# eanswer/TactileSimulation

Measured on AMD Instinct MI355X. Metric: env-steps/sec (fwd+bwd) TactilePush batch=4096, higher is better.
Workload: dtype f32

## Files before the change

### include/tsim.h

```cpp
#ifndef TSIM_H
#define TSIM_H
#include <stdint.h>
#ifdef __cplusplus
extern "C" {
#endif

typedef struct tsim_batch tsim_batch;
enum { TSIM_F32 = 0, TSIM_F64 = 1 };

int tsim_batch_create(const int32_t* I, const double* F, int B, int tape_capacity, int dtype, int device,
                      tsim_batch** out);
void tsim_batch_destroy(tsim_batch* b);

int tsim_ndof_r(const tsim_batch* b);
int tsim_ndof_u(const tsim_batch* b);
int tsim_ndof_var(const tsim_batch* b);
int tsim_ndof_tactile(const tsim_batch* b);
int tsim_batch_size(const tsim_batch* b);
int tsim_dtype(const tsim_batch* b);
double tsim_timestep(const tsim_batch* b);
int tsim_tape_len(const tsim_batch* b);

int tsim_update_model(tsim_batch* b, const int32_t* I, const double* F, void* stream);

// ... 43 lines not shown
enum { TSIM_PARAM_JACOBIAN_MAX_COLS = 32 };
int tsim_param_jacobians(tsim_batch* b, int num_frames, int num_steps, int ncols, const int32_t* cols,
                         const int32_t* tactile_slot, void* E_out, void* Ft_out, void* stream);
int tsim_param_jacobians_launch_info(const tsim_batch* b, int32_t* out);

int tsim_tactile_normal_equations(tsim_batch* b, int num_frames, int num_steps, const int32_t* tactile_slot, int with_params,
                                  const void* weight, const void* resid, void* N_out, void* n_out, void* stream);
int tsim_tactile_normal_equations_launch_info(const tsim_batch* b, int with_params, int32_t* out);

int tsim_get_adjoint(tsim_batch* b, void* df_dq0, void* df_dqd0, void* stream);

int tsim_cache_save(tsim_batch* b, void* stream);
int tsim_cache_pop(tsim_batch* b, void* stream);
int tsim_cache_clear(tsim_batch* b);
int tsim_cache_reserve(tsim_batch* b, int depth);
int tsim_cache_depth(const tsim_batch* b);

int tsim_debug_eval(tsim_batch* b, const void* q1, const void* q0, const void* qd0, const void* u,
                    void* g_out, void* H_out, long long* cycles, void* stream);

int tsim_debug_signature(tsim_batch* b, int t_first, int n, uint32_t* out, void* stream);

int tsim_debug_stamps(tsim_batch* b, long long* cycles);

int tsim_launch_info(const tsim_batch* b, int32_t* out);
enum { TSIM_KT_FORWARD = 0, TSIM_KT_TAXELS = 1, TSIM_KT_BACKWARD = 2, TSIM_KT_COUNT = 3 };
int tsim_kernel_timing(tsim_batch* b, int enable);
int tsim_kernel_times(tsim_batch* b, double* ms_sum, int32_t* launches);
int tsim_set_lanes_per_env(tsim_batch* b, int lanes);
int tsim_static_model(const tsim_batch* b);
int tsim_set_static(tsim_batch* b, int allow);
const char* tsim_kernel_variant(const tsim_batch* b);
enum { TSIM_OPT_PAIR_CULL = 1, TSIM_OPT_VALUE_TRIALS = 2, TSIM_OPT_TRIAL_HELPERS = 3, TSIM_OPT_VALUE_FIRST = 4, TSIM_OPT_CROSS_KINKS = 5, TSIM_OPT_EVAL_BUDGET = 6,
       TSIM_OPT_ALL_DEFAULT = 7, TSIM_OPT_FRAME_RECORDS = 8, TSIM_OPT_FORWARD_SPLIT = 9, TSIM_OPT_PREDICTOR_HELPERS = 10, TSIM_OPT_ADJOINT_PREPASS = 11 };
int tsim_set_option(tsim_batch* b, int option, int value);
int tsim_get_option(const tsim_batch* b, int option);

int tsim_last_evals(tsim_batch* b, int32_t* host_out);
int tsim_last_helper_trials(tsim_batch* b, int32_t* host_out);

#define TSIM_KINK_FACTOR 1000.0
#define TSIM_KINK_LS 4
#define TSIM_KINK_MAX 6
int tsim_set_solver_options(tsim_batch* b, int cross_kinks, int eval_budget);
int tsim_last_gnorm(tsim_batch* b, float* host_out);

const char* tsim_last_error(void);

#ifdef __cplusplus
}
#endif
#endif
```

### tactilesimulation_amd/csrc/tsim_batch.h

```cpp
#pragma once
#include <hip/hip_runtime.h>
#include <cstdint>
#include <string>
#include <vector>
#include "../../include/tsim.h"
#include "tsim_launch.h"

static thread_local std::string g_err;
static int fail(const std::string& m) { g_err = m; return 1; }
#define HIPCHK(x) do { hipError_t e_ = (x); if (e_ != hipSuccess) return fail(std::string(#x) + ": " + hipGetErrorString(e_)); } while (0)

struct DeviceGuard {
  int prev = -1; bool ok = true;
  explicit DeviceGuard(int dev) {
    if (hipGetDevice(&prev) != hipSuccess) prev = -1;
    if (prev != dev) ok = hipSetDevice(dev) == hipSuccess; else prev = -1;
  }
  ~DeviceGuard() { if (prev >= 0) (void)hipSetDevice(prev); }
};
#define TS_DEVICE(b) DeviceGuard guard_((b)->device); if (!guard_.ok) return fail("hipSetDevice(" + std::to_string((b)->device) + ") failed")

static bool capturing(hipStream_t st) {
  hipStreamCaptureStatus cs = hipStreamCaptureStatusNone;
  return hipStreamIsCapturing(st, &cs) != hipSuccess || cs != hipStreamCaptureStatusNone;
}

template <class F> static auto by_dtype(int dtype, F&& f) { return dtype == TSIM_F32 ? f(float()) : f(double()); }

struct DevBuf {
  void* p = nullptr;
  DevBuf() = default;
  DevBuf(const DevBuf&) = delete;
  DevBuf& operator=(const DevBuf&) = delete;
  ~DevBuf() { (void)hipFree(p); }
  template <class U> operator U*() const { return static_cast<U*>(p); }
  explicit operator bool() const { return p != nullptr; }
  void** operator&() { return &p; }
  void* take() { void* q = p; p = nullptr; return q; }
  void release() { (void)hipFree(take()); }
};

struct CacheEntry { void* buf; int len; int record, tape_k_ok; };
struct KtPair { hipEvent_t a, b; int kind; };
struct tsim_batch {
  int B, dtype, device, cap;
  std::vector<int32_t> I; std::vector<double> F;
  int nl, nr, nu, nvar, ntax, rec;
  int tape_k = 0, tape_k_ok = 0;
  DevBuf dI, dF;
  DevBuf dFenv; int nfrec;
  void* tape = nullptr;
  DevBuf lamq, lamv;
  DevBuf evals;
  DevBuf helped;
  DevBuf gnorm;
  int cross_kinks = 0, eval_budget = 0;
  DevBuf order; int order_valid = 0;
  DevBuf order_ep; int order_ep_n = 0;
  DevBuf prev; int has_prev = 0;
  DevBuf poseR, poseD; int nspt;
  int has_exp;
  int t_cur, record;
  int lpe_forced;
  int nsched;
  int stage_cpt;
  int n_simd;
  int last_frame_rec = 0;
  hipStream_t split_st = nullptr;
  hipEvent_t split_fork = nullptr;
  hipEvent_t split_join = nullptr;
  int last_fwd_split = 0;
  int value_trials = 2;
  int pred_helpers = 1;
  int trial_helpers = 1;
  int value_first = 1;
  bool ab_no_episode_lpt = false, ab_inkernel_readout = false, ab_no_free_run = false, ab_lockstep = false, ab_taxels_per_record = false, ab_no_envtab_cpt = false, ab_no_default_opts = false, ab_inkernel_frame_out = false; int ab_bwd_lpe = 0, ab_lpt_deal = 2;
  int pair_cull = 1;
  int static_id = 0, static_exact = 0, env_struct_ok = 0, no_static = 0;
  DevBuf dKmask, dFlag;
  DevBuf fposeR, fposeD; int fpose_frames = 0;
  int pose_valid = 0;
  int pose_off = 0;
  int tt_off = 0;
  int tax_slots = 0;
  size_t esz;
  std::vector<CacheEntry> cache;
// ... 59 lines not shown
```

### tactilesimulation_amd/csrc/tsim_hip.hip

```cpp
#include <hip/hip_runtime.h>
#include <cstdio>
#include <cstdlib>
#include <cstring>
#include <cmath>
#include <algorithm>
#include <string>
#include <vector>
#include "../../include/tsim.h"
#include "tsim_eval.h"
#include "tsim_policy_push.h"
#include "tsim_static_pusher.h"


#include "tsim_kernels.h"
#include "tsim_param_grad.h"
#include "tsim_launch.h"
#include "tsim_adjoint_pre.h"
#include "tsim_batch.h"

__global__ void __launch_bounds__(1024) k_order_by_evals(const int* evals, int* order, int B, int ns, int lo, int span, int deal) {
  __shared__ int hist[64], base[64];
  const int t = threadIdx.x;
  if (t < 64) hist[t] = 0;
  __syncthreads();
// ... 607 lines not shown
  HIPCHK(hipGetLastError());
  return 0;
}

template <class R>
static int launch_forward(tsim_batch* b, const void* u, int nframes, const int32_t* tac_slot, int nsub, void* q_out, void* qd_out, void* var_out, void* tac_out, int32_t* status, hipStream_t st) {
  FwdArgs<R> a = fwd_args<R>(b);
  a.nsub = nsub; a.nframes = nframes; a.tac_slot = tac_slot; a.u = (const R*)u;
  a.q_out = (R*)q_out; a.qd_out = (R*)qd_out; a.var_out = (R*)var_out; a.tac_out = (R*)tac_out; a.status = status;
  a.order = (b->B >= 256 && nframes == 1 && b->order_valid) ? (const int*)b->order : (b->B >= 256 && nframes > 1 && b->order_ep_n == nframes * nsub && !b->ab_no_episode_lpt) ? (const int*)b->order_ep : nullptr;
  a.vo_first = b->value_first; a.helpers = b->trial_helpers; a.helped = b->helped;
  a.pred_helpers = b->trial_helpers && b->pred_helpers;
  const bool emit = pose_emit(b, st);
  a.nspt = b->nspt;
  if (emit) { a.poseR = (R*)b->poseR; a.poseD = b->poseD; }
  const size_t fpose_bytes = (size_t)nframes * b->B * (size_t)std::max(b->nspt, 1) * (TP_R_SIZE * b->esz + TP_D_SIZE * sizeof(double));
  bool defer = tac_out && taxels_supported(b) && fpose_bytes <= ((size_t)1 << 30) && !b->ab_inkernel_readout;
  if (defer && b->fpose_frames < nframes) {
    if (capturing(st)) defer = false;
    else {
      const size_t nrec = (size_t)nframes * b->B * b->nspt;
      const int rc = grow_buffers(b, st, b->pose_off != 0, {{b->fposeR, nrec * TP_R_SIZE * b->esz}, {b->fposeD, nrec * TP_D_SIZE * sizeof(double)}});
      if (rc > 0) return rc;
      b->fpose_frames = rc ? 0 : nframes;
      if (rc) defer = false;
    }
  }
  if (defer) { a.fposeR = (R*)b->fposeR; a.fposeD = b->fposeD; }
  a.free_run = (defer || !tac_out || b->ntax == 0) && !b->ab_no_free_run;
  a.lockstep = b->ab_lockstep ? 1 : 0;
  if (a.lockstep) a.free_run = 0;
  TsPlan plan = ts_plan(b, TS_K_FORWARD, false, 0);
  if (b->record && !plan.fused) b->tape_k_ok = 0;
  const TsPlan fr_plan = ts_plan(b, TS_K_FRAME_RECORDS, false, 0);
  const bool frame_rec = defer && a.free_run && b->record && nframes > 1 && plan.fused && !emit && !b->ab_inkernel_frame_out &&
                         fr_plan.variant == plan.variant && fr_plan.lpe == plan.lpe;
  a.frame_rec = frame_rec ? 1 : 0;
  plan.frame_rec = frame_rec;
  b->last_frame_rec = !frame_rec ? 0 : (plan.frame_rec && plan.default_opts) ? 2 : 1;
  const int ns_ = TS_WAVE / plan.lpe;
  auto frame_records = [&](hipStream_t s, const TsSubRange& sub) {
    TsPlan p = fr_plan;
    const int nblk = (sub.n + ns_ - 1) / ns_, chunks = std::max(1, std::min(nframes, b->n_simd / std::max(nblk, 1))), fpc = (nframes + chunks - 1) / chunks;
    p.grid = (unsigned)(nblk * ((nframes + fpc - 1) / fpc));
    return ts_launch<false, R>(p, s, a, fpc, sub);
  };
  const int nblk_f = (int)plan.grid, wh = std::max(1, nblk_f / 8);
  const bool split = frame_rec && b->split_st && a.order && a.order == (const int*)b->order_ep && b->B % ns_ == 0 && nblk_f <= b->n_simd && nblk_f >= 64 &&
                     taxels_small(b, (long long)nframes * wh * ns_) && !capturing(st);
  b->last_fwd_split = split ? 1 : 0;
  if (split) {
    const TsSubRange heavy{a.order, 0, wh * ns_}, light{a.order, wh * ns_, b->B - wh * ns_};
    auto forward = [&](hipStream_t s, unsigned grid, const FwdArgs<R>& fa) -> int {
      TsPlan p = plan; p.grid = grid;
      if (!ts_launch<false, R>(p, s, fa)) return fail("no k_forward instantiation for the launch plan");
      HIPCHK(hipGetLastError());
      return 0;
    };
    auto read_out = [&](hipStream_t s, const TsSubRange& sub) -> int {
      if (!frame_records(s, sub)) return fail("no k_frame_records instantiation for the launch plan");
      HIPCHK(hipGetLastError());
      return launch_taxels<R>(b, b->fposeR, b->fposeD, nframes, tac_slot, tac_out, s, &sub);
    };
    int rc;
    {
      KtScope kt_(b, TSIM_KT_FORWARD, st);
      HIPCHK(hipEventRecord(b->split_fork, st));
      HIPCHK(hipStreamWaitEvent(b->split_st, b->split_fork, 0));
      rc = forward(st, (unsigned)wh, a);
    }
    if (!rc) {
      FwdArgs<R> al = a; al.order = a.order + light.e0;
// ... 277 lines not shown
  const int nl = I[TSIM_IH_NL], nr = I[TSIM_IH_NR], nu = I[TSIM_IH_NU];
  int n_exp = 0;
  if (nr > 16 || nr < 1 || nu > 16) return fail("ndof_r must be in 1..16 and ndof_u <= 16");
  for (int i = 1; i <= nl; ++i) {
    int jt = I[I[TSIM_IH_OFF_LINK] + (i - 1) * TSIM_LI_SIZE + TSIM_LI_JTYPE];
    if (jt != TSIM_J_REVOLUTE && jt != TSIM_J_PRISMATIC && jt != TSIM_J_PLANAR && jt != TSIM_J_TRANSLATIONAL && jt != TSIM_J_SPHERICAL_EXP)
      return fail("joint type not supported by the HIP path");
    if (jt == TSIM_J_SPHERICAL_EXP && ++n_exp > 1) return fail("at most one rotation-vector joint per model on the HIP path");
  }
  for (int s = 0; s < I[TSIM_IH_NSENSOR]; ++s)
    if (I[I[TSIM_IH_OFF_SENSOR] + s * TSIM_SI_SIZE + TSIM_SI_NSPRIM] > 16) return fail("too many primitives per sensor");
  DeviceGuard guard_(device);
  if (!guard_.ok) return fail("hipSetDevice(" + std::to_string(device) + ") failed");
  tsim_batch* b = new tsim_batch();
  b->B = B; b->dtype = dtype; b->device = device; b->cap = tape_capacity;
  b->I.assign(I, I + I[TSIM_IH_NI]); b->F.assign(F, F + I[TSIM_IH_NF]);
  b->nl = nl; b->nr = nr; b->nu = nu; b->nvar = I[TSIM_IH_NVAR]; b->ntax = I[TSIM_IH_NTAXEL];
  b->esz = dtype == TSIM_F32 ? 4 : 8;
  b->t_cur = 0; b->record = 0; b->has_exp = n_exp > 0;
  b->nfrec = I[TSIM_IH_FOFF_CPT];
  b->lpe_forced = 0;
  { const std::vector<int32_t> S_ = build_sched(b->I, b->F); b->nsched = (int)S_.size(); b->tt_off = b->I[TSIM_IH_NI] + S_[TS_SCHED_TAXTAB]; }
  b->pair_cull = getenv("TSIM_NO_PAIR_CULL") ? 0 : 1;
  b->no_static = getenv("TSIM_NO_STATIC") != nullptr;
  b->trial_helpers = getenv("TSIM_NO_TRIAL_HELPERS") ? 0 : 1;
  b->pred_helpers = getenv("TSIM_NO_PREDICTOR_HELPERS") ? 0 : 1;
  b->ab_no_episode_lpt = getenv("TSIM_NO_EPISODE_LPT") != nullptr; b->ab_inkernel_readout = getenv("TSIM_INKERNEL_READOUT") != nullptr;
  b->ab_no_free_run = getenv("TSIM_NO_FREE_RUN") != nullptr; b->ab_lockstep = getenv("TSIM_LOCKSTEP") != nullptr; b->ab_no_default_opts = getenv("TSIM_NO_DEFAULT_OPTS") != nullptr;
  if (const char* e = getenv("TSIM_LPT_DEAL")) b->ab_lpt_deal = atoi(e);
  if (const char* e = getenv("TSIM_BWD_LPE")) { const int v = atoi(e); if (v == 16 || v == 32 || v == 64) b->ab_bwd_lpe = v; }
  b->ab_taxels_per_record = getenv("TSIM_TAXELS_PER_RECORD") != nullptr; b->ab_no_envtab_cpt = getenv("TSIM_NO_ENVTAB_CPT") != nullptr;
  b->value_first = getenv("TSIM_NO_VALUE_FIRST") ? 0 : 1;
  b->ab_inkernel_frame_out = getenv("TSIM_INKERNEL_FRAME_OUT") != nullptr;
  if (const char* e = getenv("TSIM_VALUE_TRIALS")) b->value_trials = std::max(0, atoi(e));
  if (const char* e = getenv("TSIM_LPE")) { const int v = atoi(e); if (v == 16 || v == 32 || v == 64) b->lpe_forced = v; }
  b->cross_kinks = dtype == TSIM_F32 ? 1 : 0;
  {
    int cus = 0;
    if (hipDeviceGetAttribute(&cus, hipDeviceAttributeMultiprocessorCount, device) != hipSuccess || cus <= 0) cus = 256;
    b->n_simd = 4 * cus;
  }
  b->stage_cpt = 0;
  detect_static_model(b);
  b->tape_k = kernel_mode(b, b->lpe_forced) != TS_KM_GENERIC ? 1 : 0;
  b->rec = ts_rec(nr, nu, (int)b->esz, b->tape_k);
  if (lds_bytes_for(b, 1) > 64 * 1024) { delete b; return fail("model needs more than 64 KiB of LDS per environment"); }
  decide_stage_cpt(b);
  b->nspt = b->I[TSIM_IH_NSPRIM];
  size_t tape_bytes = (size_t)(tape_capacity + 1) * B * b->rec * b->esz;
  if (hipMalloc(&b->dI, (b->I.size() + b->nsched) * sizeof(int32_t)) != hipSuccess || hipMalloc(&b->dF, b->F.size() * b->esz) != hipSuccess ||
      hipMalloc(&b->tape, tape_bytes) != hipSuccess || hipMalloc(&b->lamq, (size_t)2 * B * nr * b->esz) != hipSuccess ||
      hipMalloc(&b->lamv, (size_t)2 * B * nr * b->esz) != hipSuccess || hipMalloc(&b->evals, (size_t)B * sizeof(int)) != hipSuccess || hipMalloc((void**)&b->helped, (size_t)B * sizeof(int)) != hipSuccess || hipMemset(b->helped, 0, (size_t)B * sizeof(int)) != hipSuccess || hipMalloc((void**)&b->gnorm, (size_t)B * sizeof(float)) != hipSuccess || hipMalloc(&b->order, (size_t)B * sizeof(int)) != hipSuccess || hipMalloc((void**)&b->order_ep, (size_t)B * sizeof(int)) != hipSuccess || hipMalloc(&b->prev, (size_t)B * 2 * nr * sizeof(double)) != hipSuccess ||
      (b->nspt > 0 && (hipMalloc(&b->poseR, (size_t)B * b->nspt * TP_R_SIZE * b->esz) != hipSuccess || hipMalloc((void**)&b->poseD, (size_t)B * b->nspt * TP_D_SIZE * sizeof(double)) != hipSuccess))) {
    tsim_batch_destroy(b);
    return fail("hipMalloc failed (tape bytes = " + std::to_string(tape_bytes) + ")");
  }
  if (hipMemset(b->tape, 0, tape_bytes) != hipSuccess || hipMemset(b->lamq, 0, (size_t)2 * B * nr * b->esz) != hipSuccess ||
      hipMemset(b->lamv, 0, (size_t)2 * B * nr * b->esz) != hipSuccess) { tsim_batch_destroy(b); return fail("hipMemset failed"); }
  if (upload_model(b, nullptr)) { tsim_batch_destroy(b); return 1; }
  b->adj_pre = getenv("TSIM_NO_ADJOINT_PREPASS") ? 0 : 1;
  if (b->adj_pre && b->tape_k && dtype == TSIM_F32 && tape_capacity > 0 && hipMalloc(&b->sseed, (size_t)tape_capacity * B * 2 * nr * b->esz) != hipSuccess) {
    (void)hipGetLastError();
    b->adj_pre = 0;
  }
  if (B >= 64 && !getenv("TSIM_NO_FORWARD_SPLIT")) {
    if (hipStreamCreateWithFlags(&b->split_st, hipStreamNonBlocking) != hipSuccess || hipEventCreateWithFlags(&b->split_fork, hipEventDisableTiming) != hipSuccess ||
// ... 73 lines not shown
int tsim_static_model(const tsim_batch* b) { return kernel_mode(b, b->lpe_forced) != TS_KM_GENERIC ? b->static_id : 0; }
const char* tsim_kernel_variant(const tsim_batch* b) {
  const int km = kernel_mode(b, b->lpe_forced);
  if (km == TS_KM_STATIC) return "static:pusher";
  if (km == TS_KM_PARAM) return "param:pusher";
  return "generic";
}
int tsim_set_static(tsim_batch* b, int allow) {
  b->no_static = allow ? 0 : 1;
  shape_changed(b);
  return 0;
}
int tsim_set_option(tsim_batch* b, int option, int value) {
  if (option == TSIM_OPT_PAIR_CULL) { b->pair_cull = value != 0; return 0; }
  if (option == TSIM_OPT_VALUE_TRIALS) { if (value < 0) return fail("set_option: TSIM_OPT_VALUE_TRIALS >= 0"); b->value_trials = value; return 0; }
  if (option == TSIM_OPT_TRIAL_HELPERS) { b->trial_helpers = value != 0; return 0; }
  if (option == TSIM_OPT_VALUE_FIRST) { b->value_first = value != 0; return 0; }
  if (option == TSIM_OPT_PREDICTOR_HELPERS) { b->pred_helpers = value != 0; return 0; }
  if (option == TSIM_OPT_ADJOINT_PREPASS) { b->adj_pre = value != 0; return 0; }
  return fail("set_option: unknown option " + std::to_string(option));
}
int tsim_get_option(const tsim_batch* b, int option) {
  if (option == TSIM_OPT_PAIR_CULL) return b->pair_cull;
  if (option == TSIM_OPT_VALUE_TRIALS) return b->value_trials;
  if (option == TSIM_OPT_TRIAL_HELPERS) return b->trial_helpers;
  if (option == TSIM_OPT_VALUE_FIRST) return b->value_first;
  if (option == TSIM_OPT_CROSS_KINKS) return b->cross_kinks;
  if (option == TSIM_OPT_EVAL_BUDGET) return b->eval_budget;
  if (option == TSIM_OPT_ALL_DEFAULT) return default_options(b) ? 1 : 0;
  if (option == TSIM_OPT_FRAME_RECORDS) return b->last_frame_rec;
  if (option == TSIM_OPT_FORWARD_SPLIT) return b->last_fwd_split;
  if (option == TSIM_OPT_PREDICTOR_HELPERS) return b->pred_helpers;
  if (option == TSIM_OPT_ADJOINT_PREPASS) return b->adj_pre_ran;
  return -1;
}
int tsim_set_solver_options(tsim_batch* b, int cross_kinks, int eval_budget) {
  if (eval_budget < 0) return fail("set_solver_options: negative evaluation budget");
  b->cross_kinks = cross_kinks != 0;
  b->eval_budget = eval_budget;
  return 0;
}
int tsim_last_gnorm(tsim_batch* b, float* host_out) {
  TS_DEVICE(b);
  if (hipMemcpy(host_out, b->gnorm, (size_t)b->B * sizeof(float), hipMemcpyDeviceToHost) != hipSuccess) return fail("last_gnorm: copy failed");
  return 0;
}
int tsim_last_helper_trials(tsim_batch* b, int32_t* host_out) {
  TS_DEVICE(b);
  if (hipMemcpy(host_out, b->helped, (size_t)b->B * sizeof(int), hipMemcpyDeviceToHost) != hipSuccess) return fail("last_helper_trials: copy failed");
  return 0;
}
int tsim_last_evals(tsim_batch* b, int32_t* host_out) {
  TS_DEVICE(b);
  if (hipMemcpy(host_out, b->evals, (size_t)b->B * sizeof(int), hipMemcpyDeviceToHost) != hipSuccess) return fail("last_evals: copy failed");
  return 0;
}

int tsim_update_model(tsim_batch* b, const int32_t* I, const double* F, void* stream) {
  if (I[TSIM_IH_NI] != (int)b->I.size() || I[TSIM_IH_NF] != (int)b->F.size()) return fail("update_model: blob size changed");
  for (int i = 0; i < TSIM_IH_SIZE; ++i) if (I[i] != b->I[i]) return fail("update_model: topology changed");
  TS_DEVICE(b);
  pose_invalidate(b, (hipStream_t)stream);
  b->I.assign(I, I + I[TSIM_IH_NI]); b->F.assign(F, F + I[TSIM_IH_NF]);
  if (b->dFenv) { HIPCHK(hipFree(b->dFenv)); (void)b->dFenv.take(); b->env_struct_ok = 0; }
  if (int rc = upload_model(b, (hipStream_t)stream)) return rc;
  shape_changed(b);
  return 0;
}

int tsim_set_env_tables(tsim_batch* b, const void* tables, void* stream) {
  TS_DEVICE(b);
  pose_invalidate(b, (hipStream_t)stream);
  if (!tables) { if (b->dFenv) { HIPCHK(hipFree(b->dFenv)); (void)b->dFenv.take(); b->env_struct_ok = 0; decide_stage_cpt(b); } return 0; }
  size_t bytes = (size_t)b->B * b->nfrec * b->esz;
  const bool fresh = !b->dFenv;
  if (fresh) HIPCHK(hipMalloc(&b->dFenv, bytes));
  HIPCHK(hipMemcpyAsync(b->dFenv, tables, bytes, hipMemcpyDeviceToDevice, (hipStream_t)stream));
  {
    const unsigned nh = (unsigned)((b->B * TSIM_FH_SIZE + 255) / 256);
    by_real(b, [&](auto r) { using R = decltype(r); hipLaunchKernelGGL(k_env_header<R>, dim3(nh), dim3(256), 0, (hipStream_t)stream, (R*)b->dFenv, (const R*)b->dF, b->nfrec, b->B); });
    HIPCHK(hipGetLastError());
  }
  const int ok_before = b->env_struct_ok;
  b->env_struct_ok = 0;
  if (b->static_id != 0 && b->dtype == TSIM_F32 && !capturing((hipStream_t)stream)) {
    if (!b->dKmask) {
      std::vector<unsigned char> km(b->nfrec);
// ... 338 lines not shown
```

### tactilesimulation_amd/csrc/tsim_kernels.h

```cpp
#pragma once
#include <hip/hip_runtime.h>
#include "../../include/tsim.h"
#include "tsim_eval.h"
#include "tsim_policy_push.h"

template <class MS, class C> __device__ __forceinline__ int ts_integrator(const C& c) {
  if constexpr (std::is_void<MS>::value) return ts_u(c.I[TSIM_IH_INTEGRATOR]); else return MS::Iv(TSIM_IH_INTEGRATOR);
}
template <class MS> constexpr int ts_static_nr() { if constexpr (std::is_void<MS>::value) return 0; else return MS::Iv(TSIM_IH_NR); }

__host__ __device__ inline int ts_qw(int esz) { return 8 / esz; }
__host__ __device__ inline int ts_rec(int nr, int nu, int esz, int tk) { return (ts_qw(esz) * nr + nr + nr * nr + nu + (tk ? nr * nr : 0) + 1) & ~1; }
template <class R> __device__ __forceinline__ double* rec_q(R* rec) { return reinterpret_cast<double*>(rec); }
template <class R> __device__ __forceinline__ const double* rec_q(const R* rec) { return reinterpret_cast<const double*>(rec); }
template <class R> __device__ __forceinline__ int rec_qd(int nr) { return ts_qw((int)sizeof(R)) * nr; }
template <class R> __device__ __forceinline__ int rec_H(int nr) { return ts_qw((int)sizeof(R)) * nr + nr; }
template <class R> __device__ __forceinline__ int rec_u(int nr) { return ts_qw((int)sizeof(R)) * nr + nr + nr * nr; }
template <class R> __device__ __forceinline__ int rec_K(int nr, int nu) { return ts_qw((int)sizeof(R)) * nr + nr + nr * nr + nu; }

template <int LPE, class R>
__device__ __forceinline__ void readout(const Ctx<R>& c, int lane, int env, bool wr_var, bool wr, bool has_var, bool has_tac, R* var_out, R* tac_out, int tb = 0, int te = 0x7fffffff) {
  if (has_var && wr_var) {
    for (int e = lane; e < c.nvar; e += LPE) {
      const int l = c.I[c.off_var + e * TSIM_VI_SIZE + TSIM_VI_LINK];
      const V3<R> x = mulMv(ldm(c.LP + l * LK_SIZE + LK_R), ldv(c.F + c.foff_var + e * TSIM_VF_SIZE)) + ldv(c.LP + l * LK_SIZE + LK_P);
      R* o = var_out + (size_t)env * 3 * c.nvar + 3 * e;
      o[0] = x.x; o[1] = x.y; o[2] = x.z;
    }
  }
  if (!has_tac) return;
  for (int s = 0; s < c.nsensor; ++s) {
    const int* si = c.I + c.off_sensor + s * TSIM_SI_SIZE;
    const R* sf = c.F + c.foff_sensor + s * TSIM_SF_SIZE;
    const int t0 = ts_u(si[TSIM_SI_TAX0]), nt = ts_u(si[TSIM_SI_NTAX]), sp0 = ts_u(si[TSIM_SI_SPRIM0]), nsp = ts_u(si[TSIM_SI_NSPRIM]);
    for (int j0 = 0; j0 < nsp || j0 == 0; j0 += TS_PAIR_GROUP) {
      const int je = min(j0 + TS_PAIR_GROUP, nsp);
      TS_SYNC();
      for (int j = j0; j < je; ++j) pair_stage_value(c, ts_u(c.I[c.off_sprim + sp0 + j]), j - j0, lane == 0);
      TS_SYNC();
      const int lo = max(tb, t0) - t0, hi = min(te, t0 + nt) - t0;
      for (int base = lo; base < hi; base += LPE) {
        const int t = t0 + base + lane;
        if (base + lane >= hi || !wr) continue;
        const R* tp = c.Fg + c.foff_tax + t;
        const V3<R> xa = mk3<R>(tp[0], tp[c.ntax], tp[2 * c.ntax]);
// ... 40 lines not shown
};
__device__ __forceinline__ unsigned ts_drop_lowest(unsigned mask, int n, int nmax) {
  for (int i = 0; i < nmax; ++i) { if (i < n) mask &= mask - 1u; }
  return mask;
}
enum { TP_R_SIZE = 18, TP_D_SIZE = 12 };
struct TsSubRange { const int* order; int e0, n; };
template <class R> struct FwdArgs {
  const int* I; const R* F; const R* Fenv; int fstride;
  int B, nsub, record, t0;
  int tk = 0;
  int nframes;
  const int* tac_slot;
  R* tape; const R* u;
  R *q_out, *qd_out, *var_out, *tac_out; int* status; int* evals;
  const int* order;
  double* prev; int has_prev;
  int stage_cpt;
  int cross_kinks;
  int eval_budget;
  float* gnorm;
  PushPolicy<R> pol;
  R* poseR = nullptr; double* poseD = nullptr; int nspt = 0;
  int free_run = 0;
  int lockstep = 0;
  R* fposeR = nullptr; double* fposeD = nullptr;
  int cull = 0;
  int vo_ls = 0;
  int* helped = nullptr;
  int vo_first = 0;
  int default_opts = 0;
  int helpers = 0;
  int frame_rec = 0;
  int pred_helpers = 0;
};

template <int LPE, class R, class MS>
__device__ __forceinline__ void ts_frame_outputs(const Ctx<R>& c, const FwdArgs<R>& a, int lane, int env, int f, int tslot, bool frame_end, bool valid) {
  const int nr = c.nr;
  if constexpr (ts_static_fused<MS, R>()) { if (frame_end) ts_static_value_records<R, MS>(c, lane); }
  if (frame_end && lane < nr && valid) {
    const size_t o = ((size_t)f * a.B + env) * nr + lane;
    if (a.q_out) a.q_out[o] = (R)c.q0D[lane];
    if (a.qd_out) a.qd_out[o] = c.qd0[lane];
  }
  const bool tac_here = a.tac_out != nullptr && !a.fposeR;
  readout<LPE>(c, lane, env, frame_end && valid, frame_end && valid && tslot >= 0, a.var_out != nullptr, tac_here && tslot >= 0,
               a.var_out ? a.var_out + (size_t)f * a.B * 3 * c.nvar : nullptr,
               (tac_here && tslot >= 0) ? a.tac_out + (size_t)tslot * a.B * 3 * c.ntax : nullptr);
  if (a.fposeR && frame_end && tslot >= 0) {
    int k = 0;
    for (int sn = 0; sn < c.nsensor; ++sn) {
      const int* si = c.I + c.off_sensor + sn * TSIM_SI_SIZE;
      const int nsp = ts_u(si[TSIM_SI_NSPRIM]), sp0 = ts_u(si[TSIM_SI_SPRIM0]);
      for (int j = 0; j < nsp; ++j, ++k) {
        TS_SYNC();
        pair_stage_value(c, ts_u(c.I[c.off_sprim + sp0 + j]), 0, lane == 0);
        TS_SYNC();
        const size_t rec = ((size_t)f * a.B + env) * a.nspt + k;
        if (valid) {
          for (int e = lane; e < TP_R_SIZE; e += LPE) a.fposeR[rec * TP_R_SIZE + e] = c.PP[e];
          if (lane < TP_D_SIZE) a.fposeD[rec * TP_D_SIZE + lane] = c.PPd[lane];
        }
      }
    }
  }
// ... 288 lines not shown
        if (vfirst && ls >= 0) kq = (ls == 0 && !forced && gn > R(0)) ? gtake / (gn * gn) : R(1e30);
        forced = false;
        if (ls >= 0) ++iter;
        gn = gtake;
        if (!ts_finite(gn)) { nonfinite = true; fin = true; }
        else if (gn < c.tol) { conv = true; fin = true; }
        else if (iter >= c.max_iter || (TS_OPT(eval_budget, 0) > 0 && sub_evals >= TS_OPT(eval_budget, 0))) fin = true;
        else {
          solve = true;
          if (lane < nr) { c.rhs[lane] = -c.g[lane]; dlbase[lane] = c.dl[lane]; }
        }
      }
    }
    TS_SYNC();
    if constexpr (!kPred) { TS_NEWTON_STEPS }
    bool commit = fin && !done && !held;
    if (TS_OPT(lockstep, 0) && !__all(fin || done)) commit = false;
    if (!free_run) {
      if (commit && s == a.nsub - 1) { held = true; commit = false; }
      if (__all(held || done)) { commit = held; held = false; }
    }
    bool frame_end = false;
    if (commit) {
#ifdef TS_ROUND_STATS
      if (hround_ && !(s == a.nsub - 1 && f == a.nframes - 1)) { ++hc_; if (hserved_) ++hcs_; }
#endif
      if (!conv) ++bad;
      gmax = t_max(gmax, gn);
      if (TS_RECORD && valid) {
        R* rec = a.tape + ((size_t)(a.t0 + f * a.nsub + s + 1) * a.B + env) * REC;
        if (lane < nr) { rec_q(rec)[lane] = c.qD[lane]; rec[rec_qd<R>(nr) + lane] = c.qd[lane]; }
        for (int e = lane; e < nr * nr; e += LPE) rec[rec_H<R>(nr) + e] = c.H[e];
        if (lane < nu) rec[rec_u<R>(nr) + lane] = c.u[lane];
        if constexpr (ts_static_fused<MS, R>()) { if (a.tk) for (int e = lane; e < nr * nr; e += LPE) rec[rec_K<R>(nr, nu) + e] = c.H2[e]; }
      }
      TS_SYNC();
      if (lane < nr) {
        c.qm1[lane] = c.q0[lane]; c.qm1D[lane] = c.q0D[lane]; c.qdm1[lane] = c.qd0[lane];
        c.q0[lane] = c.q[lane]; c.q0D[lane] = c.qD[lane]; c.qd0[lane] = c.qd[lane];
      }
      has_prev = true;
      fin = false; ss = true;
      if (++s == a.nsub) { s = 0; frame_end = true; }
    }
    TS_SYNC();
    if constexpr (kPred) {
      if (TS_UNLIKELY(__any(po.hp >= 0 && commit))) {
        if (po.hp >= 0 && commit) {
          c.cv = R(1) / c.h; c.ca = R(1) / (c.h * c.h);
          if (lane < nr) { c.qpD[lane] = ts_predictor_bdf1(c.q0D[lane], c.h, c.qd0[lane]); c.qp[lane] = (R)c.qpD[lane]; c.qdp[lane] = c.qd0[lane]; c.dl[lane] = R(0); }
          alpha = R(1); iter = 0; ls = -1; crossings = 0; conv = false; forced = false; vo = false; ss = false;
          const int d = (po.hp - slot) * ts_lds_env_reals(c.nl, nr, nu, (int)sizeof(R));
          if (lane < nr) c.g[lane] = c.g[lane + d];
          for (int e = lane; e < nr * nr; e += LPE) { c.H[e] = c.H[e + d]; c.H2[e] = c.H2[e + d]; }
          ++evals; sub_evals = 1; ++helped;
          gn = po.gp; fin = true;
          if (!ts_finite(gn)) nonfinite = true;
          else if (gn < c.tol) conv = true;
          else if (!(iter >= c.max_iter || (TS_OPT(eval_budget, 0) > 0 && sub_evals >= TS_OPT(eval_budget, 0)))) {
            fin = false; solve = true;
            if (lane < nr) { c.rhs[lane] = -c.g[lane]; dlbase[lane] = c.dl[lane]; }
          }
        }
        TS_SYNC();
      }
      TS_NEWTON_STEPS
    }
    if constexpr (kFrameRec) {
      if (frame_end) { ++f; fs = true; if (f == a.nframes) { done = true; fs = false; ss = false; } }
    } else if (TS_UNLIKELY(__any(frame_end))) {
#ifdef TS_ROUND_STATS
      ++fe_execs_; const long long fe_t0_ = clock64();
#endif
      if (!(ts_static_fused<MS, R>() && !POLICY && a.frame_rec != 0)) ts_frame_outputs<LPE, R, MS>(c, a, lane, env, f, tslot, frame_end, valid);
      if (frame_end) { ++f; fs = true; if (f == a.nframes) { done = true; fs = false; ss = false; } }
      TS_SYNC();
// ... 37 lines not shown
    if (lane == 0) { if (a.gnorm) a.gnorm[env] = (float)(clock64() - rs_t0_); if (a.status) a.status[env] = rounds_; }
    if (lane == 0 && a.helped) a.helped[env] = (int)(fe_cycles_ < (1ll << 23) - 1 ? fe_cycles_ : (1ll << 23) - 1) * 256 + (fe_execs_ < 255 ? fe_execs_ : 255);
    if (kFrameRec && lane == 0 && a.helped) a.helped[env] = min(hr_, 2047) | min(hc_, 1023) << 11 | min(hcs_, 1023) << 21;
#endif
  }
}
#undef helpers_on
#undef pred_on
#undef pred_need
#undef TS_NEWTON_STEPS
#undef TS_OPT
#undef TS_RECORD
template <class R, int NRM, bool EXPJ, int LPE, bool POLICY = false, class MS = void>
__global__ void TS_KLB k_forward(FwdArgs<R> a) { ts_forward<R, NRM, EXPJ, LPE, POLICY, MS>(a); }
template <class R, int NRM, int LPE, class MS>
__global__ void TS_KLB k_forward_fr(FwdArgs<R> a) { ts_forward<R, NRM, false, LPE, false, TsFrameRecords<TsDefaultOpts<MS>>>(a); }

template <class R, int LPE, class MS>
__global__ void TS_KLB k_frame_records(FwdArgs<R> a, int fpc, TsSubRange sub) {
  extern __shared__ __attribute__((aligned(16))) unsigned char smem_raw[];
  R* lds = reinterpret_cast<R*>(smem_raw);
  constexpr int NS = TS_WAVE / LPE;
  const int slot = threadIdx.x / LPE, lane = threadIdx.x % LPE;
  const int nblk = (sub.n + NS - 1) / NS, chunk = blockIdx.x / nblk;
  const int eidx = (blockIdx.x - chunk * nblk) * NS + slot;
  const bool valid = eidx < sub.n;
  const int ei = sub.e0 + min(eidx, sub.n - 1);
  const int env = sub.order ? sub.order[ei] : ei;
  Ctx<R> c; ctx_init<R, MS>(c, a.I, a.F, lds, NS, slot, lane, LPE, false, a.Fenv ? a.Fenv + (size_t)env * a.fstride : nullptr);
  const int nr = c.nr, REC = ts_rec(nr, c.nu, (int)sizeof(R), a.tk);
  init_world(c, lane, LPE);
  const int f0 = chunk * fpc, f1 = min(f0 + fpc, a.nframes);
  double qn = 0.0; R qdn = R(0);
  const R* st = a.tape + ((size_t)(a.t0 + (f0 + 1) * a.nsub) * a.B + env) * REC;
  const size_t frame_stride = (size_t)a.nsub * a.B * REC;
  if (f0 < f1 && lane < nr) { qn = rec_q(st)[lane]; qdn = st[rec_qd<R>(nr) + lane]; }
  for (int f = f0; f < f1; ++f) {
    const int tslot = a.tac_slot ? a.tac_slot[f] : f;
    TS_SYNC();
    if (lane < nr) { c.qD[lane] = qn; c.q0D[lane] = qn; c.q[lane] = (R)qn; c.qd[lane] = qdn; c.qd0[lane] = qdn; c.qa[lane] = R(0); }
    st += frame_stride;
    if (f + 1 < f1 && lane < nr) { qn = rec_q(st)[lane]; qdn = st[rec_qd<R>(nr) + lane]; }
    TS_SYNC();
    ts_frame_outputs<LPE, R, MS>(c, a, lane, env, f, tslot, true, valid);
  }
}


template <class R, int LPE, class MS> __device__ __forceinline__ void ts_static_output_vjp(const Ctx<R>& c, int lane, const R* wvar, const R* wtac);
template <class R> struct BwdArgs {
  const int* I; const R* F; const R* Fenv; int fstride;
  int B, n, t_end;
  int tk = 0;
  int seed_stride;
  int frames;
  const int* tac_slot;
  const R* tape;
  const R *df_dq, *df_dvar, *df_dtac;
  R *lamq, *lamv, *df_du;
  int stage_cpt;
  long long* cyc;
  PushPolicy<R> pol;
  int cull = 0;
};

template <int LPE, class R>
__device__ __forceinline__ R mass_times_z(const Ctx<R>& c, int lane) {
  const int* LR = c.LI + ts_sched_rec(c.LI);
  R* fi = c.PT;
  for (int i = 1 + lane; i <= c.nl; i += LPE) {
    const int anc = LR[(i - 1) * TS_LR_SIZE + TS_LR_ANCMASK];
    S6<R> A = zero6<R>();
    for (int k = 0; k < c.nr; ++k)
      if ((anc >> k) & 1) A = A + ld6(c.WP + k * 6) * c.z[k];
    const R* X = c.LP + i * LK_SIZE;
// ... 247 lines not shown
```

### tactilesimulation_amd/host/batch.py

```python
import ctypes as C

import numpy as np
import torch

from . import capi
from ..model import blob as _blob
from ..model.compiler import CompiledModel, load_model


def _ptr(t):
    return C.c_void_p(t.data_ptr()) if t is not None else None


class BatchSim:
    def __init__(self, model, batch_size, device="cuda:0", dtype=torch.float32, tape_capacity=512):
        if isinstance(model, str):
            model = load_model(model)
        assert isinstance(model, CompiledModel)
        self.model = model
        self.device = torch.device(device)
        if self.device.type != "cuda":
            raise RuntimeError("BatchSim needs a GPU device (got %s); the HIP path has no CPU fallback" % device)
        if dtype not in (torch.float32, torch.float64):
            raise ValueError("dtype must be float32 or float64")
# ... 298 lines not shown

    def cache_pop(self):
        capi.check(capi.lib().tsim_cache_pop(self._h, self._stream()))

    def cache_clear(self):
        capi.check(capi.lib().tsim_cache_clear(self._h))

    def cache_reserve(self, depth):
        capi.check(capi.lib().tsim_cache_reserve(self._h, int(depth)))

    def cache_depth(self):
        return capi.lib().tsim_cache_depth(self._h)

    def debug_eval(self, q1, q0, qd0, u, cycles=False):
        q1, q0, qd0 = (self._chk(x, self.ndof_r, "q") for x in (q1, q0, qd0))
        u = self._chk(u, self.ndof_u, "u")
        g, H = self.empty(self.ndof_r), self.empty(self.ndof_r, self.ndof_r)
        cyc = torch.zeros(self.B, 32, device=self.device, dtype=torch.int64) if cycles else None
        capi.check(capi.lib().tsim_debug_eval(self._h, _ptr(q1), _ptr(q0), _ptr(qd0), _ptr(u), _ptr(g), _ptr(H), _ptr(cyc),
                                              self._stream()))
        return (g, H, cyc) if cycles else (g, H)

    def branch_signature(self, t_first=0, n=None):
        n = self.tape_len() - t_first if n is None else int(n)
        out = torch.empty((n, self.B, 2), device=self.device, dtype=torch.int32)
        capi.check(capi.lib().tsim_debug_signature(self._h, int(t_first), n, _ptr(out), self._stream()))
        return out.to(torch.int64) & 0xFFFFFFFF

    def last_evals(self):
        out = np.zeros(self.B, dtype=np.int32)
        capi.check(capi.lib().tsim_last_evals(self._h, out.ctypes.data_as(capi._ip)))
        return out

    def last_helper_trials(self):
        out = np.zeros(self.B, dtype=np.int32)
        capi.check(capi.lib().tsim_last_helper_trials(self._h, out.ctypes.data_as(capi._ip)))
        return out

    def last_gnorm(self):
        out = np.zeros(self.B, dtype=np.float32)
        capi.check(capi.lib().tsim_last_gnorm(self._h, out.ctypes.data_as(C.POINTER(C.c_float))))
        return out

    def set_solver_options(self, cross_kinks=None, eval_budget=0):
        if cross_kinks is None:
            cross_kinks = self.dtype == torch.float32
        capi.check(capi.lib().tsim_set_solver_options(self._h, int(bool(cross_kinks)), int(eval_budget)))

    def set_lanes_per_env(self, lanes):
        capi.check(capi.lib().tsim_set_lanes_per_env(self._h, int(lanes)))

    def static_model(self):
        return capi.lib().tsim_static_model(self._h)

    def set_static(self, allow):
        capi.check(capi.lib().tsim_set_static(self._h, int(bool(allow))))

    def kernel_variant(self):
        return capi.lib().tsim_kernel_variant(self._h).decode()

    OPT_PAIR_CULL, OPT_VALUE_TRIALS, OPT_TRIAL_HELPERS, OPT_VALUE_FIRST, OPT_CROSS_KINKS, OPT_EVAL_BUDGET, OPT_ALL_DEFAULT, OPT_FRAME_RECORDS = 1, 2, 3, 4, 5, 6, 7, 8
    OPT_FORWARD_SPLIT = 9
    OPT_PREDICTOR_HELPERS = 10
    OPT_ADJOINT_PREPASS = 11

    def set_option(self, option, value):
        capi.check(capi.lib().tsim_set_option(self._h, int(option), int(value)))

    def get_option(self, option):
        return capi.lib().tsim_get_option(self._h, int(option))

    KERNEL_KINDS = ("k_forward", "k_taxels", "k_backward")

    def kernel_timing(self, enable=True):
        capi.check(capi.lib().tsim_kernel_timing(self._h, int(bool(enable))))

    def kernel_times(self):
        ms, n = (C.c_double * 3)(), (C.c_int32 * 3)()
        capi.check(capi.lib().tsim_kernel_times(self._h, ms, n))
        return {k: (float(ms[i]), int(n[i])) for i, k in enumerate(self.KERNEL_KINDS)}

    def launch_info(self):
        out = (C.c_int32 * 4)()
        capi.lib().tsim_launch_info(self._h, out)
        return {"lds_bytes": out[0], "threads": out[1], "blocks": out[2], "lanes_per_env": out[3]}

    def tangent_launch_info(self, ndir=8, with_dtables=True):
        out = (C.c_int32 * 4)()
        capi.check(capi.lib().tsim_tangent_launch_info(self._h, int(ndir), int(bool(with_dtables)), out))
        return {"lds_bytes": out[0], "threads": out[1], "blocks": out[2], "lanes_per_env": out[3]}

    def frame_jacobians_launch_info(self):
        out = (C.c_int32 * 4)()
        capi.check(capi.lib().tsim_frame_jacobians_launch_info(self._h, out))
        return {"lds_bytes": out[0], "threads": out[1], "blocks": out[2], "lanes_per_env": out[3]}

    def tactile_jacobians_launch_info(self):
        out = (C.c_int32 * 4)()
# ... 13 lines not shown
```

### tactilesimulation_amd/host/capi.py

```python
import ctypes as C
import os

_DIR = os.path.join(os.path.dirname(os.path.abspath(__file__)), "..", "csrc")
LIB_PATH = os.environ.get("TSIM_HIP_LIB") or os.path.abspath(os.path.join(_DIR, "libtsim_hip.so"))
_lib = None

TSIM_F32, TSIM_F64 = 0, 1
_vp, _ip = C.c_void_p, C.POINTER(C.c_int32)

_SIGS = {
    "tsim_batch_create": (C.c_int, [_ip, C.POINTER(C.c_double), C.c_int, C.c_int, C.c_int, C.c_int, C.POINTER(_vp)]),
    "tsim_batch_destroy": (None, [_vp]),
    "tsim_ndof_r": (C.c_int, [_vp]), "tsim_ndof_u": (C.c_int, [_vp]), "tsim_ndof_var": (C.c_int, [_vp]),
    "tsim_ndof_tactile": (C.c_int, [_vp]), "tsim_batch_size": (C.c_int, [_vp]), "tsim_dtype": (C.c_int, [_vp]),
    "tsim_timestep": (C.c_double, [_vp]), "tsim_tape_len": (C.c_int, [_vp]),
    "tsim_update_model": (C.c_int, [_vp, _ip, C.POINTER(C.c_double), _vp]),
    "tsim_reset": (C.c_int, [_vp, _vp, _vp, C.c_int, _vp]),
    "tsim_set_env_tables": (C.c_int, [_vp, _vp, _vp]), "tsim_table_size": (C.c_int, [_vp]),
    "tsim_set_param_grad": (C.c_int, [_vp, _vp]),
    "tsim_set_param_grad_groups": (C.c_int, [_vp, C.c_int]), "tsim_get_param_grad_groups": (C.c_int, [_vp]),
    "tsim_reset_masked": (C.c_int, [_vp, _vp, _vp, _vp, _vp]),
    "tsim_step": (C.c_int, [_vp, _vp, C.c_int, _vp, _vp, _vp, _vp, _vp, _vp]),
    "tsim_get_state": (C.c_int, [_vp, _vp, _vp, _vp]),
    "tsim_readout": (C.c_int, [_vp, _vp, _vp, _vp]),
    "tsim_backward_steps": (C.c_int, [_vp, C.c_int, C.c_int, _vp, _vp, _vp, _vp, _vp]),
    "tsim_rollout": (C.c_int, [_vp, _vp, C.c_int, C.c_int, _vp, _vp, _vp, _vp, _vp, _vp, _vp]),
    "tsim_backward_episode": (C.c_int, [_vp, C.c_int, C.c_int, _vp, _vp, _vp, _vp, _vp, _vp]),
    "tsim_get_adjoint": (C.c_int, [_vp, _vp, _vp, _vp]),
    "tsim_tangent_episode": (C.c_int, [_vp, C.c_int, C.c_int, C.c_int, _vp, _vp, _vp, _vp, _vp, _vp, _vp, _vp, _vp, _vp]),
    "tsim_cache_save": (C.c_int, [_vp, _vp]), "tsim_cache_pop": (C.c_int, [_vp, _vp]), "tsim_cache_clear": (C.c_int, [_vp]),
    "tsim_cache_reserve": (C.c_int, [_vp, C.c_int]), "tsim_cache_depth": (C.c_int, [_vp]),
    "tsim_debug_signature": (C.c_int, [_vp, C.c_int, C.c_int, _vp, _vp]),
    "tsim_debug_eval": (C.c_int, [_vp, _vp, _vp, _vp, _vp, _vp, _vp, _vp, _vp]),
    "tsim_debug_stamps": (C.c_int, [_vp, _vp]),
    "tsim_launch_info": (C.c_int, [_vp, _ip]),
    "tsim_tangent_launch_info": (C.c_int, [_vp, C.c_int, C.c_int, _ip]),
    "tsim_frame_jacobians": (C.c_int, [_vp, C.c_int, C.c_int, _vp, _vp, _vp, _vp]),
    "tsim_frame_jacobians_launch_info": (C.c_int, [_vp, _ip]),
    "tsim_tactile_jacobians": (C.c_int, [_vp, C.c_int, C.c_int, _vp, _vp, _vp]),
    "tsim_tactile_jacobians_launch_info": (C.c_int, [_vp, _ip]),
    "tsim_param_jacobians": (C.c_int, [_vp, C.c_int, C.c_int, C.c_int, _ip, _vp, _vp, _vp, _vp]),
    "tsim_param_jacobians_launch_info": (C.c_int, [_vp, _ip]),
    "tsim_tactile_normal_equations": (C.c_int, [_vp, C.c_int, C.c_int, _vp, C.c_int, _vp, _vp, _vp, _vp, _vp]),
    "tsim_tactile_normal_equations_launch_info": (C.c_int, [_vp, C.c_int, _ip]),
    "tsim_last_adjoint_launch": (C.c_int, [_vp, _ip]),
    "tsim_set_lanes_per_env": (C.c_int, [_vp, C.c_int]),
    "tsim_kernel_timing": (C.c_int, [_vp, C.c_int]), "tsim_kernel_times": (C.c_int, [_vp, C.POINTER(C.c_double), _ip]),
    "tsim_static_model": (C.c_int, [_vp]), "tsim_set_static": (C.c_int, [_vp, C.c_int]),
    "tsim_kernel_variant": (C.c_char_p, [_vp]),
    "tsim_set_option": (C.c_int, [_vp, C.c_int, C.c_int]), "tsim_get_option": (C.c_int, [_vp, C.c_int]),
    "tsim_last_evals": (C.c_int, [_vp, _ip]),
    "tsim_last_helper_trials": (C.c_int, [_vp, _ip]),
    "tsim_set_solver_options": (C.c_int, [_vp, C.c_int, C.c_int]),
    "tsim_last_gnorm": (C.c_int, [_vp, C.POINTER(C.c_float)]),
    "tsim_last_error": (C.c_char_p, []),
    "tsim_model_load": (C.c_int, [C.c_char_p, C.POINTER(_vp)]), "tsim_model_free": (None, [_vp]),
    "tsim_model_blob": (C.c_int, [_vp, C.POINTER(_ip), C.POINTER(C.c_int), C.POINTER(C.POINTER(C.c_double)), C.POINTER(C.c_int)]),
    "tsim_model_save_blob": (C.c_int, [_vp, C.c_char_p]), "tsim_model_load_blob": (C.c_int, [C.c_char_p, C.POINTER(_vp)]),
    "tsim_batch_create_from_model": (C.c_int, [_vp, C.c_int, C.c_int, C.c_int, C.c_int, C.POINTER(_vp)]),
    "tsim_model_image_pos": (C.c_int, [_vp, C.c_char_p, _ip, C.c_int]),
    "tsim_model_update": (C.c_int, [_vp, C.c_int, C.c_char_p, C.c_char_p, C.POINTER(C.c_double), C.c_int]),
    "tsim_model_table_offset": (C.c_int, [_vp, C.c_int, C.c_char_p, C.c_char_p, C.c_int]),
    "tsim_push_action": (C.c_int, [C.c_int, C.c_int, _vp, _vp, _vp, _vp]),
    "tsim_push_action_backward": (C.c_int, [C.c_int, C.c_int, _vp, _vp, _vp, _vp]),
    "tsim_push_observe": (C.c_int, [C.c_int, C.c_int, C.c_int, _vp, _vp, _vp, _vp, _vp, _vp, _vp, _vp]),
    "tsim_push_closed_rollout": (C.c_int, [_vp, _vp, _vp, _vp, _vp, C.c_int, C.c_int, _vp, _vp, _vp, _vp, _vp, _vp, _vp, _vp, _vp, _vp]),
    "tsim_push_closed_backward": (C.c_int, [_vp, _vp, _vp, C.c_int, C.c_int, _vp, _vp, _vp, _vp, _vp, _vp, _vp, _vp, _vp, _vp, _vp, _vp]),
    "tsim_push_closed_tangent": (C.c_int, [_vp, _vp, _vp, C.c_int, C.c_int, C.c_int] + [_vp] * 18),
    "tsim_push_closed_tangent_launch_info": (C.c_int, [_vp, C.c_int, C.c_int, _ip]),
    "tsim_push_observe_backward": (C.c_int, [C.c_int, C.c_int, C.c_int, _vp, _vp, _vp, _vp, _vp, _vp, C.c_longlong, _vp, _vp, _vp, _vp, _vp]),
}
EXPORTS = sorted(_SIGS)


class PushPolicyStruct(C.Structure):
    _fields_ = [(n, C.c_void_p) for n in ("W1T", "b1", "W2T", "b2", "W3", "b3", "W1p", "W2")] + [("w1_stride", C.c_int), ("obs_mode", C.c_int)] + \
               [(n, C.c_void_p) for n in ("eps", "logstd", "obs_mean", "obs_istd")] + [("obs_clip", C.c_double)]


def lib():
    global _lib
    if _lib is None:
        if not os.path.exists(LIB_PATH):
            raise RuntimeError("HIP extension not built: %s is missing (run `python -c 'import __graft_entry__ as g; "
# ... 36 lines not shown
```

Baseline: 36.99 million.

## Profile per-frame solver evals and reorder envs by measured episode cost

Records each environment's per-frame Newton evaluation count into a grown evals buffer, either directly at frame end or through a padding slot in the fused frame records. On later rollouts with a full profile, it launches k_order_by_evals to build an LPT-style environment ordering from the accumulated costs. This balances work across wavefronts and cores by grouping environments with similar iteration counts. In exchange it adds per-frame global writes, a one-time synchronize and reallocation to grow the buffer, and a small ordering kernel on each rollout.

Measured after the change: 36.78 million. No clear change (-0.6%).

```diff
diff --git a/include/tsim.h b/include/tsim.h
--- a/include/tsim.h
+++ b/include/tsim.h
@@ -99,11 +99,14 @@
 int tsim_set_static(tsim_batch* b, int allow);
 const char* tsim_kernel_variant(const tsim_batch* b);
 enum { TSIM_OPT_PAIR_CULL = 1, TSIM_OPT_VALUE_TRIALS = 2, TSIM_OPT_TRIAL_HELPERS = 3, TSIM_OPT_VALUE_FIRST = 4, TSIM_OPT_CROSS_KINKS = 5, TSIM_OPT_EVAL_BUDGET = 6,
-       TSIM_OPT_ALL_DEFAULT = 7, TSIM_OPT_FRAME_RECORDS = 8, TSIM_OPT_FORWARD_SPLIT = 9, TSIM_OPT_PREDICTOR_HELPERS = 10, TSIM_OPT_ADJOINT_PREPASS = 11 };
+       TSIM_OPT_ALL_DEFAULT = 7, TSIM_OPT_FRAME_RECORDS = 8, TSIM_OPT_FORWARD_SPLIT = 9, TSIM_OPT_PREDICTOR_HELPERS = 10, TSIM_OPT_ADJOINT_PREPASS = 11,
+       TSIM_OPT_PROFILE_ORDER = 12, TSIM_OPT_PROFILE_ROWS = 13 };
 int tsim_set_option(tsim_batch* b, int option, int value);
 int tsim_get_option(const tsim_batch* b, int option);
 
 int tsim_last_evals(tsim_batch* b, int32_t* host_out);
+int tsim_episode_profile(tsim_batch* b, int first_row, int nrows, int32_t* host_out);
+int tsim_episode_order(tsim_batch* b, int32_t* host_out, int32_t* n);
 int tsim_last_helper_trials(tsim_batch* b, int32_t* host_out);
 
 #define TSIM_KINK_FACTOR 1000.0
diff --git a/tactilesimulation_amd/csrc/tsim_batch.h b/tactilesimulation_amd/csrc/tsim_batch.h
--- a/tactilesimulation_amd/csrc/tsim_batch.h
+++ b/tactilesimulation_amd/csrc/tsim_batch.h
@@ -52,6 +52,8 @@
   void* tape = nullptr;
   DevBuf lamq, lamv;
   DevBuf evals;
+  int evals_rows = 0, prof_rows = 0, prof_nsub = 0, prof_on = 1;
+  int last_prof_order = 0;
   DevBuf helped;
   DevBuf gnorm;
   int cross_kinks = 0, eval_budget = 0;
diff --git a/tactilesimulation_amd/csrc/tsim_hip.hip b/tactilesimulation_amd/csrc/tsim_hip.hip
--- a/tactilesimulation_amd/csrc/tsim_hip.hip
+++ b/tactilesimulation_amd/csrc/tsim_hip.hip
@@ -663,12 +663,33 @@
   if (a.lockstep) a.free_run = 0;
   TsPlan plan = ts_plan(b, TS_K_FORWARD, false, 0);
   if (b->record && !plan.fused) b->tape_k_ok = 0;
+  b->last_prof_order = 0;
+  const bool prof = b->prof_on && nframes > 1 && !capturing(st);
+  if (prof) {
+    if (b->prof_nsub != nsub) { b->prof_rows = 0; b->prof_nsub = nsub; }
+    if (b->evals_rows < nframes && !b->pose_off && (long long)(1 + nframes) * b->B < (1ll << 31)) {
+      HIPCHK(hipStreamSynchronize(st));
+      void* grown = nullptr;
+      if (hipMalloc(&grown, (size_t)(1 + nframes) * b->B * sizeof(int)) != hipSuccess) (void)hipGetLastError();
+      else if (hipMemcpy(grown, b->evals, (size_t)(1 + b->prof_rows) * b->B * sizeof(int), hipMemcpyDeviceToDevice) != hipSuccess) { (void)hipGetLastError(); (void)hipFree(grown); }
+      else { b->evals.release(); b->evals.p = grown; b->evals_rows = nframes; a.evals = b->evals; }
+    }
+    if (b->evals_rows >= nframes && (long long)(1 + nframes) * b->B < (1ll << 31)) a.evals_rows = nframes;
+    if (!a.order && b->prof_rows >= nframes && b->B >= 256 && !b->ab_no_episode_lpt) {
+      const int ns = TS_WAVE / plan.lpe, nsv = (b->B % ns == 0) ? ns : 1, n = nframes * nsub;
+      hipLaunchKernelGGL(k_order_by_evals, dim3(1), dim3(1024), 0, st, (const int*)b->evals + (size_t)nframes * b->B, b->order_ep, b->B, nsv, 2 * n, std::max(1, 5 * n / 2), b->ab_lpt_deal);
+      HIPCHK(hipGetLastError());
+      b->order_ep_n = n; a.order = (const int*)b->order_ep; b->last_prof_order = 1;
+    }
+  }
   const TsPlan fr_plan = ts_plan(b, TS_K_FRAME_RECORDS, false, 0);
   const bool frame_rec = defer && a.free_run && b->record && nframes > 1 && plan.fused && !emit && !b->ab_inkernel_frame_out &&
                          fr_plan.variant == plan.variant && fr_plan.lpe == plan.lpe;
   a.frame_rec = frame_rec ? 1 : 0;
   plan.frame_rec = frame_rec;
   b->last_frame_rec = !frame_rec ? 0 : (plan.frame_rec && plan.default_opts) ? 2 : 1;
+  if (b->last_frame_rec == 2 && a.evals_rows) { if (b->tape_k && b->esz == 4 && ts_rec_pad(b->nr, b->nu, 4, 1)) a.evals_pad = 1; else a.evals_rows = 0; }
+  if (a.evals_rows) b->prof_rows = std::max(b->prof_rows, nframes);
   const int ns_ = TS_WAVE / plan.lpe;
   auto frame_records = [&](hipStream_t s, const TsSubRange& sub) {
     TsPlan p = fr_plan;
@@ -1012,6 +1033,7 @@
   b->ab_taxels_per_record = getenv("TSIM_TAXELS_PER_RECORD") != nullptr; b->ab_no_envtab_cpt = getenv("TSIM_NO_ENVTAB_CPT") != nullptr;
   b->value_first = getenv("TSIM_NO_VALUE_FIRST") ? 0 : 1;
   b->ab_inkernel_frame_out = getenv("TSIM_INKERNEL_FRAME_OUT") != nullptr;
+  b->prof_on = getenv("TSIM_NO_PROFILE_ORDER") ? 0 : 1;
   if (const char* e = getenv("TSIM_VALUE_TRIALS")) b->value_trials = std::max(0, atoi(e));
   if (const char* e = getenv("TSIM_LPE")) { const int v = atoi(e); if (v == 16 || v == 32 || v == 64) b->lpe_forced = v; }
   b->cross_kinks = dtype == TSIM_F32 ? 1 : 0;
@@ -1151,6 +1173,8 @@
   if (option == TSIM_OPT_FORWARD_SPLIT) return b->last_fwd_split;
   if (option == TSIM_OPT_PREDICTOR_HELPERS) return b->pred_helpers;
   if (option == TSIM_OPT_ADJOINT_PREPASS) return b->adj_pre_ran;
+  if (option == TSIM_OPT_PROFILE_ORDER) return b->last_prof_order;
+  if (option == TSIM_OPT_PROFILE_ROWS) return b->prof_rows;
   return -1;
 }
 int tsim_set_solver_options(tsim_batch* b, int cross_kinks, int eval_budget) {
@@ -1172,6 +1196,19 @@
 int tsim_last_evals(tsim_batch* b, int32_t* host_out) {
   TS_DEVICE(b);
   if (hipMemcpy(host_out, b->evals, (size_t)b->B * sizeof(int), hipMemcpyDeviceToHost) != hipSuccess) return fail("last_evals: copy failed");
+  return 0;
+}
+int tsim_episode_profile(tsim_batch* b, int first_row, int nrows, int32_t* host_out) {
+  if (first_row < 1 || nrows < 0 || first_row + nrows - 1 > b->prof_rows) return fail("episode_profile: rows " + std::to_string(first_row) + " .. " + std::to_string(first_row + nrows - 1) + " of " + std::to_string(b->prof_rows));
+  if (nrows == 0) return 0;
+  TS_DEVICE(b);
+  if (hipMemcpy(host_out, (const int*)b->evals + (size_t)first_row * b->B, (size_t)nrows * b->B * sizeof(int), hipMemcpyDeviceToHost) != hipSuccess) return fail("episode_profile: copy failed");
+  return 0;
+}
+int tsim_episode_order(tsim_batch* b, int32_t* host_out, int32_t* n) {
+  TS_DEVICE(b);
+  if (hipMemcpy(host_out, b->order_ep, (size_t)b->B * sizeof(int), hipMemcpyDeviceToHost) != hipSuccess) return fail("episode_order: copy failed");
+  *n = b->order_ep_n;
   return 0;
 }
 
diff --git a/tactilesimulation_amd/csrc/tsim_kernels.h b/tactilesimulation_amd/csrc/tsim_kernels.h
--- a/tactilesimulation_amd/csrc/tsim_kernels.h
+++ b/tactilesimulation_amd/csrc/tsim_kernels.h
@@ -11,6 +11,7 @@
 
 __host__ __device__ inline int ts_qw(int esz) { return 8 / esz; }
 __host__ __device__ inline int ts_rec(int nr, int nu, int esz, int tk) { return (ts_qw(esz) * nr + nr + nr * nr + nu + (tk ? nr * nr : 0) + 1) & ~1; }
+__host__ __device__ inline bool ts_rec_pad(int nr, int nu, int esz, int tk) { return ((ts_qw(esz) * nr + nr + nr * nr + nu + (tk ? nr * nr : 0)) & 1) != 0; }
 template <class R> __device__ __forceinline__ double* rec_q(R* rec) { return reinterpret_cast<double*>(rec); }
 template <class R> __device__ __forceinline__ const double* rec_q(const R* rec) { return reinterpret_cast<const double*>(rec); }
 template <class R> __device__ __forceinline__ int rec_qd(int nr) { return ts_qw((int)sizeof(R)) * nr; }
@@ -117,6 +118,8 @@
   int default_opts = 0;
   int helpers = 0;
   int frame_rec = 0;
+  int evals_rows = 0;
+  int evals_pad = 0;
   int pred_helpers = 0;
 };
 
@@ -471,7 +474,12 @@
         if (lane < nr) { rec_q(rec)[lane] = c.qD[lane]; rec[rec_qd<R>(nr) + lane] = c.qd[lane]; }
         for (int e = lane; e < nr * nr; e += LPE) rec[rec_H<R>(nr) + e] = c.H[e];
         if (lane < nu) rec[rec_u<R>(nr) + lane] = c.u[lane];
-        if constexpr (ts_static_fused<MS, R>()) { if (a.tk) for (int e = lane; e < nr * nr; e += LPE) rec[rec_K<R>(nr, nu) + e] = c.H2[e]; }
+        if constexpr (ts_static_fused<MS, R>()) {
+          if (a.tk) {
+            for (int e = lane; e < nr * nr; e += LPE) rec[rec_K<R>(nr, nu) + e] = c.H2[e];
+            if constexpr (kFrameRec && sizeof(R) == 4) { if (lane == 0 && ts_rec_pad(nr, nu, 4, 1)) rec[rec_K<R>(nr, nu) + nr * nr] = __int_as_float(evals); }
+          }
+        }
       }
       TS_SYNC();
       if (lane < nr) {
@@ -480,7 +488,10 @@
       }
       has_prev = true;
       fin = false; ss = true;
-      if (++s == a.nsub) { s = 0; frame_end = true; }
+      if (++s == a.nsub) {
+        s = 0; frame_end = true;
+        if constexpr (!kFrameRec) { if (TS_UNLIKELY(f < a.evals_rows) && valid && lane == 0) a.evals[(f + 1) * a.B + env] = evals; }
+      }
     }
     TS_SYNC();
     if constexpr (kPred) {
@@ -584,15 +595,20 @@
   init_world(c, lane, LPE);
   const int f0 = chunk * fpc, f1 = min(f0 + fpc, a.nframes);
   double qn = 0.0; R qdn = R(0);
+  int evn = 0;
+  const bool prof = sizeof(R) == 4 && a.evals_pad != 0 && valid && lane == 0;
   const R* st = a.tape + ((size_t)(a.t0 + (f0 + 1) * a.nsub) * a.B + env) * REC;
   const size_t frame_stride = (size_t)a.nsub * a.B * REC;
   if (f0 < f1 && lane < nr) { qn = rec_q(st)[lane]; qdn = st[rec_qd<R>(nr) + lane]; }
+  if (f0 < f1 && prof) evn = __float_as_int((float)st[rec_K<R>(nr, c.nu) + nr * nr]);
   for (int f = f0; f < f1; ++f) {
     const int tslot = a.tac_slot ? a.tac_slot[f] : f;
+    if (prof && f < a.evals_rows) a.evals[(f + 1) * a.B + env] = evn;
     TS_SYNC();
     if (lane < nr) { c.qD[lane] = qn; c.q0D[lane] = qn; c.q[lane] = (R)qn; c.qd[lane] = qdn; c.qd0[lane] = qdn; c.qa[lane] = R(0); }
     st += frame_stride;
     if (f + 1 < f1 && lane < nr) { qn = rec_q(st)[lane]; qdn = st[rec_qd<R>(nr) + lane]; }
+    if (f + 1 < f1 && prof) evn = __float_as_int((float)st[rec_K<R>(nr, c.nu) + nr * nr]);
     TS_SYNC();
     ts_frame_outputs<LPE, R, MS>(c, a, lane, env, f, tslot, true, valid);
   }
diff --git a/tactilesimulation_amd/host/batch.py b/tactilesimulation_amd/host/batch.py
--- a/tactilesimulation_amd/host/batch.py
+++ b/tactilesimulation_amd/host/batch.py
@@ -354,6 +354,17 @@
         capi.check(capi.lib().tsim_last_evals(self._h, out.ctypes.data_as(capi._ip)))
         return out
 
+    def episode_profile(self, first_row=1, nrows=None):
+        nrows = self.get_option(self.OPT_PROFILE_ROWS) - int(first_row) + 1 if nrows is None else int(nrows)
+        out = np.zeros((max(nrows, 0), self.B), dtype=np.int32)
+        capi.check(capi.lib().tsim_episode_profile(self._h, int(first_row), nrows, out.ctypes.data_as(capi._ip)))
+        return out
+
+    def episode_order(self):
+        out, n = np.zeros(self.B, dtype=np.int32), C.c_int32(0)
+        capi.check(capi.lib().tsim_episode_order(self._h, out.ctypes.data_as(capi._ip), C.byref(n)))
+        return out, int(n.value)
+
     def last_helper_trials(self):
         out = np.zeros(self.B, dtype=np.int32)
         capi.check(capi.lib().tsim_last_helper_trials(self._h, out.ctypes.data_as(capi._ip)))
@@ -386,6 +397,8 @@
     OPT_PREDICTOR_HELPERS = 10
     OPT_ADJOINT_PREPASS = 11
 
+    OPT_PROFILE_ORDER, OPT_PROFILE_ROWS = 12, 13
+
     def set_option(self, option, value):
         capi.check(capi.lib().tsim_set_option(self._h, int(option), int(value)))
 
diff --git a/tactilesimulation_amd/host/capi.py b/tactilesimulation_amd/host/capi.py
--- a/tactilesimulation_amd/host/capi.py
+++ b/tactilesimulation_amd/host/capi.py
@@ -50,6 +50,7 @@
     "tsim_kernel_variant": (C.c_char_p, [_vp]),
     "tsim_set_option": (C.c_int, [_vp, C.c_int, C.c_int]), "tsim_get_option": (C.c_int, [_vp, C.c_int]),
     "tsim_last_evals": (C.c_int, [_vp, _ip]),
+    "tsim_episode_profile": (C.c_int, [_vp, C.c_int, C.c_int, _ip]), "tsim_episode_order": (C.c_int, [_vp, _ip, _ip]),
     "tsim_last_helper_trials": (C.c_int, [_vp, _ip]),
     "tsim_set_solver_options": (C.c_int, [_vp, C.c_int, C.c_int]),
     "tsim_last_gnorm": (C.c_int, [_vp, C.POINTER(C.c_float)]),
```
